# Lab-LVM/imagenet-models

Hardware: AMD Instinct MI355X
Metric: images/sec (whole node) GA-ConvNeXt-T 3x224x224 bf16 training step (higher is better)
Workload: dtype bf16; 1 GPU; ga_convnext_tiny_768 train step (fwd + GA loss lam=-0.8 + bwd + all-reduce + adamw lr=0), batch 256/GPU, drop_path 0.2, synthetic 3x224x224; global_batch=256, parallelism=dp1, dist_backend=none, grad_exchange=torch, allreduce_buckets=0

## Files before the change

imagenet-models_amd/_lib.py:

```python
import ctypes as C
import os

_HERE = os.path.dirname(os.path.abspath(__file__))
LIB_PATH = os.environ.get('GAEXT_LIB') or os.path.join(_HERE, 'csrc', 'libgaext.so')

GA_F32, GA_BF16 = 0, 1
ACT_NONE, ACT_GELU, ACT_RELU = 0, 1, 2
A_PLAIN, A_PATCH2, A_STEM4_NCHW, A_CONV3, A_CONV3S2, A_NEIGH2 = 0, 1, 2, 3, 4, 5
C_PLAIN, C_UNPATCH2 = 0, 1

vp, i32, i64, f32 = C.c_void_p, C.c_int, C.c_int64, C.c_float


class GemmDesc(C.Structure):
    _fields_ = [
        ('M', i32), ('N', i32), ('K', i32), ('batch', i32), ('dtype', i32),
        ('A', vp), ('lda', i64), ('strideA', i64), ('a_batch_mod', i32), ('a_kind', i32),
        ('a_H', i32), ('a_W', i32), ('a_C', i32), ('a_act', i32),
        ('B', vp), ('ldb', i64), ('strideB', i64),
        ('C', vp), ('ldc', i64), ('strideC', i64), ('c_kind', i32),
        ('c_H', i32), ('c_W', i32), ('c_C', i32), ('c_f32', i32), ('C2', vp), ('c2_mode', i32),
        ('alpha', f32), ('bias', vp), ('strideBias', i64), ('act', i32),
        ('H', vp), ('ldh', i64), ('strideH', i64), ('h_is_deriv', i32),
        ('rowscale', vp), ('rows_per_scale', i32),
# ... 173 lines not shown
    'ga_loss_dense_fwd_bwd': ([vp, vp, vp, vp, vp, vp, vp, i32, i32, i32, f32, i32, f32, f32, f32, i32, vp], i32),
    'ga_u8_normalize': ([vp, vp, i32, i32, i32, i32, C.POINTER(f32), C.POINTER(f32), vp], i32),
    'ga_input_erase': ([vp, i32, vp, i32, i32, i32, i32, C.POINTER(f32), C.POINTER(f32), vp, i32, i32, C.c_uint64, C.c_uint64, vp], i32),
    'ga_input_collate': ([vp, i32, vp, i32, i32, i32, i32, C.POINTER(f32), C.POINTER(f32), vp, vp, i32, i32, C.c_uint64, C.c_uint64, vp],
                         i32),
    'ga_mixup_target_elem': ([vp, vp, i32, i32, vp, C.c_double, vp], i32),
    'ga_mixup_batch': ([vp, vp, i32, i32, i32, i32, C.c_double, i32, i32, i32, i32, i32, vp], i32),
    'ga_mixup_target': ([vp, vp, i32, i32, C.c_double, C.c_double, vp], i32),
    'ga_agc_clip': ([vp, vp, vp, i32, f32, f32, vp], i32),
    'ga_small_linear_fwd': ([C.POINTER(SmallLinearDesc), vp], i32),
    'ga_small_linear_bwd': ([C.POINTER(SmallLinearDesc), vp, vp, i32, vp, vp, vp, vp], i32),
    'ga_colstats': ([vp, i64, i32, i32, vp, vp, i32, vp], i32),
    'ga_pad_copy_f32': ([vp, vp, i64, i64, i64, i64, i32, vp], i32),
    'ga_pad_copy': ([vp, vp, i64, i64, i64, i64, i32, i32, vp], i32),
    'ga_stem4_ln_fwd': ([vp, vp, i64, vp, vp, vp, vp, vp, vp, vp, i32, i32, i32, i32, f32, vp], i32),
    'ga_blockdiag_f32': ([vp, vp, i64, i32, i32, i32, i64, i32, i32, vp], i32),
    'ga_pad_groups_f32': ([vp, vp, i64, i64, i32, i32, i32, i32, i32, i32, vp], i32),
    'ga_attn_fwd': ([C.POINTER(AttnDesc), vp], i32),
    'ga_attn_bwd_workspace': ([C.POINTER(AttnDesc)], C.c_size_t),
    'ga_attn_bwd': ([C.POINTER(AttnDesc), vp, vp, vp, C.c_size_t, vp], i32),
    'ga_patchify': ([vp, vp, i32, i32, i32, i32, i32, i32, vp], i32),
    'ga_vit_embed_fwd': ([vp, vp, vp, vp, i32, i32, i32, i32, vp], i32),
    'ga_vit_embed_bwd': ([vp, vp, vp, vp, i32, i32, i32, i32, vp], i32),
    'ga_patchify_strided': ([vp, vp, i32, i32, i32, i32, i32, i32, i32, vp], i32),
    'ga_pos_add_fwd': ([vp, vp, vp, i32, i32, i32, i32, vp], i32),
    'ga_pos_add_bwd': ([vp, vp, i32, i32, i32, i32, vp], i32),
    'ga_dwpool_fwd': ([vp, vp, vp, vp, i32, i32, i32, i32, i32, i32, vp], i32),
    'ga_dwpool_bwd_data': ([vp, vp, vp, i32, i32, i32, i32, i32, i32, vp], i32),
    'ga_dwpool_bwd_weight': ([vp, vp, vp, vp, i32, i32, i32, i32, i32, i32, vp], i32),
    'ga_resize_concat_fwd': ([vp, vp, i32, i32, i32, i32, i32, i32, i64, i32, i32, vp], i32),
    'ga_resize_concat_bwd': ([vp, vp, i32, i32, i32, i32, i32, i32, i64, i32, i32, vp], i32),
    'ga_rows_bcast': ([vp, vp, i32, i32, i32, f32, i32, vp], i32),
    'ga_token_gap_fwd': ([vp, vp, i32, i32, i32, i32, vp], i32),
    'ga_token_gap_bwd': ([vp, vp, i32, i32, i32, i32, vp], i32),
    'ga_mlp_supported': ([i32, i32, i32], i32),
    'ga_mlp_fwd': ([C.POINTER(MlpDesc), vp], i32),
    'ga_mlp_bwd': ([C.POINTER(MlpBwdDesc), vp], i32),
    'ga_mlp_bwd_wgrad_supported': ([i32, i32, i32], i32),
    'ga_mlp_bwd_partials': ([C.POINTER(MlpBwdDesc)], C.c_size_t),
    'ga_memset': ([vp, i32, C.c_size_t, vp], i32),
    'ga_transpose_f32': ([vp, vp, i32, i32, i32, vp], i32),
    'ga_axpy_f32': ([vp, vp, f32, i64, vp], i32),
    'ga_lerp_f32': ([vp, vp, f32, i64, vp], i32),
    'ga_sumsq_f32': ([vp, i64, vp, vp], i32),
    'ga_lamb_stage1': ([vp, vp, vp, vp, vp, vp, vp, vp, i32, vp, vp], i32),
    'ga_lamb_stage2': ([vp, vp, vp, vp, i32, vp, vp], i32),
    'ga_clip_grad_f32': ([vp, i64, vp, f32, i32, vp], i32),
    'ga_rowscale': ([vp, vp, vp, i64, i64, i32, vp], i32),
    'ga_cast_from_f32': ([vp, vp, i64, i32, vp], i32),
    'ga_cast_to_f32': ([vp, vp, i64, i32, vp], i32),
}

_lib = None


def load():
    global _lib
    if _lib is not None:
        return _lib
    if not os.path.exists(LIB_PATH):
        raise RuntimeError(f'libgaext.so not found at {LIB_PATH}: build it with `make -C {os.path.dirname(LIB_PATH)}` '
                           f'(there is no CPU fallback for the product path)')
    lib = C.CDLL(LIB_PATH)
    for name, (argtypes, restype) in _SIGS.items():
        fn = getattr(lib, name)
        fn.argtypes = argtypes
        fn.restype = restype
    _lib = lib
    return lib


def last_error():
    buf = C.create_string_buffer(512)
    load().ga_last_error(buf, 512)
    return buf.value.decode(errors='replace')


def config_string():
    buf = C.create_string_buffer(1024)
    load().ga_config_string(buf, 1024)
    s = buf.value.decode(errors='replace')
    host = sorted(k for k in os.environ if k.startswith(('GAEXT_', 'GA_FUSED_MLP')) and k != 'GAEXT_LIB')
    known = {'GAEXT_ASYNC_WGRAD', 'GAEXT_FWD_SPLIT', 'GAEXT_PAR_BRANCH', 'GAEXT_FWD_SKEW', 'GAEXT_FUSE_DP', 'GAEXT_HEAD_STREAMS',
             'GA_FUSED_MLP', 'GAEXT_SMALL_SINGLE', 'GAEXT_SYNC_DEBUG', 'GAEXT_MLP_WG1'}
    for k in host:
        if k in known:
            s += f' host:{k}={os.environ[k]}'
    if os.environ.get('GAEXT_LIB'):
        s += f' lib={os.environ["GAEXT_LIB"]}'
    return s


class knobs:

    def __init__(self, **kv):
        self.kv = kv

    def __enter__(self):
        lib = load()
        for k, v in self.kv.items():
            check(lib.ga_set_knob(k.encode(), int(v)), f'ga_set_knob({k})')
        return self

    def __exit__(self, *exc):
        lib = load()
        for k in self.kv:
            lib.ga_unset_knob(k.encode())
        return False


def check(rc, what):
    if rc != 0:
        raise RuntimeError(f'libgaext {what} failed (code {rc}): {last_error()}')


def exported_symbols():
    return sorted(_SIGS)
```

imagenet-models_amd/csrc/gemm.hip:

```cpp
#include <stdlib.h>
#include <algorithm>
#include <type_traits>
#include "common.h"

namespace {

int num_cus() {
    static int n = [] {
        int c = 256;
        ga_device_info(&c, nullptr, nullptr);
        return c;
    }();
    return n;
}

constexpr int kThreads = 256;
constexpr int kRowBytes = 128;

__device__ __forceinline__ int xcd_remap(int bid, int nwg) {
    const int q = nwg >> 3, r = nwg & 7, xcd = bid & 7, idx = bid >> 3;
    return (xcd < r ? xcd * (q + 1) : r * (q + 1) + (xcd - r) * q) + idx;
}

struct RowCtx {
// ... 1471 lines not shown
        const int cur = (int)((s - s_begin) & 1);
        if (s + 1 < s_end) g_load(s + 1);
        const unsigned char* Ys = smem + cur * 32768;
        const unsigned char* Xs = Ys + 16384;
        if constexpr (sizeof(T) == 2) {
#pragma unroll
            for (int ks = 0; ks < 2; ++ks) {
                s16x4_t yf[4][2], xf[4][2];
#pragma unroll
                for (int hf = 0; hf < 2; ++hf) {
                    const int row = ks * 32 + 8 * (lane >> 4) + 4 * hf + ((lane & 15) >> 2);
                    const int sw = tn_swz(row);
#pragma unroll
                    for (int t = 0; t < 4; ++t) {
                        const int ch_y = ((wn * 64 + t * 16) >> 3) + ((lane & 3) >> 1);
                        const int ch_x = ((wk * 64 + t * 16) >> 3) + ((lane & 3) >> 1);
                        const unsigned ay = row * P::RB + ((ch_y ^ sw) << 4) + 8 * (lane & 1);
                        const unsigned ax = row * P::RB + ((ch_x ^ sw) << 4) + 8 * (lane & 1);
                        yf[t][hf] = __builtin_amdgcn_ds_read_tr16_b64_v4i16(
                            (__attribute__((address_space(3))) s16x4_t*)(Ys + ay));
                        xf[t][hf] = __builtin_amdgcn_ds_read_tr16_b64_v4i16(
                            (__attribute__((address_space(3))) s16x4_t*)(Xs + ax));
                    }
                }
#pragma unroll
                for (int tn = 0; tn < 4; ++tn)
#pragma unroll
                    for (int tk = 0; tk < 4; ++tk)
                        acc[tn][tk] = __builtin_amdgcn_mfma_f32_16x16x32_bf16(
                            *reinterpret_cast<const bf16x8_t*>(&yf[tn][0]), *reinterpret_cast<const bf16x8_t*>(&xf[tk][0]),
                            acc[tn][tk], 0, 0, 0);
            }
        } else {
#pragma unroll
            for (int ks = 0; ks < 8; ++ks) {
                const int row = ks * 4 + (lane >> 4);
                float yf[4], xf[4];
#pragma unroll
                for (int t = 0; t < 4; ++t) {
                    yf[t] = *reinterpret_cast<const float*>(Ys + row * P::RB + (wn * 64 + t * 16 + (lane & 15)) * 4);
                    xf[t] = *reinterpret_cast<const float*>(Xs + row * P::RB + (wk * 64 + t * 16 + (lane & 15)) * 4);
                }
#pragma unroll
                for (int tn = 0; tn < 4; ++tn)
#pragma unroll
                    for (int tk = 0; tk < 4; ++tk)
                        acc[tn][tk] = __builtin_amdgcn_mfma_f32_16x16x4f32(yf[tn], xf[tk], acc[tn][tk], 0, 0, 0);
            }
        }
        if (s + 1 < s_end) s_store(cur ^ 1);
        __syncthreads();
    }

    float* W = d.dW + z * d.strideW;
    const bool atomic = d.accumulate || d.split_m > 1;
#pragma unroll
    for (int tn = 0; tn < 4; ++tn)
#pragma unroll
        for (int tk = 0; tk < 4; ++tk)
#pragma unroll
            for (int r = 0; r < 4; ++r) {
                const int n = n0 + wn * 64 + tn * 16 + (lane >> 4) * 4 + r;
                const int k = k0 + wk * 64 + tk * 16 + (lane & 15);
                if (n < d.N && k < d.K) {
                    const float v = acc[tn][tk][r] * d.alpha;
                    if (atomic) atomicAdd(W + (long)n * d.ldw + k, v);
                    else W[(long)n * d.ldw + k] = v;
                }
            }
    if (do_bias) {
        float* red = reinterpret_cast<float*>(smem);
#pragma unroll
        for (int j = 0; j < EPC; ++j) red[rr * 128 + cc * EPC + j] = bsum[j];
        __syncthreads();
        if (tid < 128 && n0 + tid < d.N) {
            float s = 0.f;
            for (int r = 0; r < P::RSTEP; ++r) s += red[r * 128 + tid];
            atomicAdd(d.dbias + z * d.strideDbias + n0 + tid, s * d.alpha);
        }
    }
}

constexpr int kTn2Threads = 512, kTn2Stage = 32768, kTn2Smem = 4 * kTn2Stage;

template <bool P2>
__global__ __launch_bounds__(kTn2Threads) void gemm_tn2_kernel(const ga_wgrad_desc d, const int split_m,
                                                               float* __restrict__ part) {
    extern __shared__ __attribute__((aligned(16))) unsigned char smem[];
    const int tid = threadIdx.x, lane = tid & 63;
    const int wave = __builtin_amdgcn_readfirstlane(tid >> 6);
    const int wn = wave >> 2, wk = wave & 3;
    const int tiles_k = (d.K + 255) / 256, tiles_n = (d.N + 255) / 256;
    const int ntiles = tiles_k * tiles_n;
    const int bid = xcd_remap(blockIdx.x, ntiles * split_m);
    const int split = bid / ntiles, tile = bid - split * ntiles;
    const int tile_n = tile / tiles_k, tile_k = tile - tile_n * tiles_k;
    const int n0 = tile_n * 256, k0 = tile_k * 256;
    const int z = blockIdx.z;
    const int stages = d.M / 32;
    const int per = (stages + split_m - 1) / split_m;
    const int s_begin = split * per;
    const int s_end = s_begin + per < stages ? s_begin + per : stages;
    if (s_begin >= s_end) return;

    const int sub = wave >> 1;
    const bool is_y = sub < 2;
    const int ncols = is_y ? d.N : d.K;
    const int col0 = (is_y ? n0 : k0) + (sub & 1) * 128;
    const bool sub_live = col0 < ncols;
    const long ld = is_y ? d.ldy : d.ldx;
    const int zx = d.x_batch_mod > 0 ? z % d.x_batch_mod : z;
    const bf16_t* gsrc = is_y ? reinterpret_cast<const bf16_t*>(d.Y) + z * d.strideY
                              : reinterpret_cast<const bf16_t*>(d.X) + zx * d.strideX;
    const int lrow = 16 * (wave & 1) + (lane >> 4);
    const int pc = lane & 15;
    const bool xp2 = P2 && !is_y;
    const int sw_lo = ((lane >> 4) & 3) << 1;
    long goff[2];
#pragma unroll
    for (int b = 0; b < 2; ++b) {
        int c = col0 + ((pc ^ (sw_lo | (b << 3))) << 3);
        if (c >= ncols) c = 0;
        if (xp2) goff[b] = c + (c >= 2 * d.x_C ? (long)(d.x_W - 2) * d.x_C : 0);
        else goff[b] = (long)lrow * ld + c;
    }
    const unsigned lds0 = (unsigned)(size_t)(__attribute__((address_space(3))) unsigned char*)smem;
    const u32x4_s rs = make_rsrc(gsrc, xp2 ? (unsigned)(8L * d.M * d.x_C) : 0xffffffffu);
    unsigned voff[4];
    [[maybe_unused]] unsigned p2_ox[4];
    [[maybe_unused]] unsigned p2_ow = 1, p2_r = 0, p2_step = 0, p2_carry = 0;
    if (xp2) {
        p2_ow = (unsigned)d.x_W >> 1;
        const unsigned q = 32u / p2_ow, rowb = (unsigned)(d.x_W * d.x_C) * 2u;
        p2_r = 32u - q * p2_ow;
        p2_step = 128u * (unsigned)d.x_C + q * rowb;
        p2_carry = rowb;
#pragma unroll
        for (int i = 0; i < 4; ++i) {
            const unsigned m = (unsigned)s_begin * 32u + (unsigned)(lrow + 4 * i), t = m / p2_ow;
            p2_ox[i] = m - t * p2_ow;
            voff[i] = (unsigned)(((long)(2u * m + (unsigned)d.x_W * t)) * d.x_C + goff[(i >> 1) & 1]) * 2u;
        }
    } else {
#pragma unroll
        for (int i = 0; i < 4; ++i) voff[i] = (unsigned)(goff[(i >> 1) & 1] + (long)(4 * i) * ld) * 2u;
    }
    auto stage_load = [&](int s, int buf) __attribute__((always_inline)) {
        if (!sub_live) return;
        const unsigned soff = xp2 ? 0u : (unsigned)s * 64u * (unsigned)ld;
        const unsigned dst = lds0 + buf * kTn2Stage + sub * 8192 + (wave & 1) * 4096;
#pragma unroll
        for (int i = 0; i < 4; ++i) blds16(rs, voff[i], soff, dst + i * 1024);
        if constexpr (P2) {
            if (xp2) {
#pragma unroll
                for (int i = 0; i < 4; ++i) {
                    p2_ox[i] += p2_r;
                    const bool carry = p2_ox[i] >= p2_ow;
                    p2_ox[i] -= carry ? p2_ow : 0u;
                    voff[i] += p2_step + (carry ? p2_carry : 0u);
                }
            }
        }
    };

    int nv = (d.N - n0 - wn * 128 + 15) / 16; nv = nv < 0 ? 0 : (nv > 8 ? 8 : nv);
    int kv = (d.K - k0 - wk * 64 + 15) / 16;  kv = kv < 0 ? 0 : (kv > 4 ? 4 : kv);
    const bool do_bias = d.dbias != nullptr && tile_k == 0 && wk == 0;
    f32x4_t acc[8][4];
    float bsum[8];
#pragma unroll
    for (int i = 0; i < 8; ++i) {
        bsum[i] = 0.f;
#pragma unroll
        for (int j = 0; j < 4; ++j) acc[i][j] = f32x4_t{0.f, 0.f, 0.f, 0.f};
    }
    typedef __attribute__((ext_vector_type(2))) __bf16 bf16x2_t;
    const bf16x2_t ones2 = {(__bf16)1.0f, (__bf16)1.0f};

    const unsigned y_img = wn * 8192, x_img = 16384 + (wk >> 1) * 8192;
    const int xc0 = (wk & 1) * 8;
    unsigned yaddr[8], xaddr[4];
    {
        const int row = 8 * (lane >> 4) + ((lane & 15) >> 2);
        const int sw = tn_swz(row);
        const unsigned rb = row * 256 + 8 * (lane & 1);
#pragma unroll
        for (int t = 0; t < 8; ++t) yaddr[t] = y_img + rb + (((2 * t + ((lane & 3) >> 1)) ^ sw) << 4);
#pragma unroll
        for (int t = 0; t < 4; ++t) xaddr[t] = x_img + rb + (((xc0 + 2 * t + ((lane & 3) >> 1)) ^ sw) << 4);
    }
    auto compute = [&](int cur) {
        const unsigned char* st = smem + cur * kTn2Stage;
        s16x4_t yf[8][2], xf[4][2];
#pragma unroll
        for (int hf = 0; hf < 2; ++hf) {
#pragma unroll
            for (int t = 0; t < 4; ++t)
                xf[t][hf] = __builtin_amdgcn_ds_read_tr16_b64_v4i16(
                    (__attribute__((address_space(3))) s16x4_t*)(st + xaddr[t] + hf * 1024));
#pragma unroll
            for (int t = 0; t < 8; ++t)
                yf[t][hf] = __builtin_amdgcn_ds_read_tr16_b64_v4i16(
                    (__attribute__((address_space(3))) s16x4_t*)(st + yaddr[t] + hf * 1024));
        }
#pragma unroll
        for (int tn = 0; tn < 8; ++tn) {
            const bf16x8_t a = *reinterpret_cast<const bf16x8_t*>(&yf[tn][0]);
#pragma unroll
            for (int tk = 0; tk < 4; ++tk)
                acc[tn][tk] = __builtin_amdgcn_mfma_f32_16x16x32_bf16(
                    a, *reinterpret_cast<const bf16x8_t*>(&xf[tk][0]), acc[tn][tk], 0, 0, 0);
        }
        if (do_bias) {
#pragma unroll
            for (int tn = 0; tn < 8; ++tn) {
                const bf16x8_t a = *reinterpret_cast<const bf16x8_t*>(&yf[tn][0]);
#pragma unroll
                for (int j = 0; j < 4; ++j)
                    bsum[tn] = __builtin_amdgcn_fdot2_f32_bf16(bf16x2_t{a[2 * j], a[2 * j + 1]}, ones2, bsum[tn], false);
            }
        }
    };

    const int nst = s_end - s_begin;
#pragma unroll
    for (int j = 0; j < 3; ++j)
        if (j < nst) stage_load(s_begin + j, j);
    for (int it = 0; it < nst; ++it) {
        const int ahead = nst - 1 - it;
        if (ahead >= 2) asm volatile("s_waitcnt vmcnt(8)" ::: "memory");
        else if (ahead == 1) asm volatile("s_waitcnt vmcnt(4)" ::: "memory");
        else asm volatile("s_waitcnt vmcnt(0)" ::: "memory");
        __builtin_amdgcn_s_barrier();
        if (it + 3 < nst) stage_load(s_begin + it + 3, (it + 3) & 3);
        if (nv > 0 && kv > 0) compute(it & 3);
    }

    float* W = part ? part + ((long)z * split_m + split) * d.N * d.K : d.dW + z * d.strideW;
    const long ldw = part ? d.K : d.ldw;
    const float alpha = part ? 1.f : d.alpha;
    const bool atomic = !part && (d.accumulate || split_m > 1);
#pragma unroll
    for (int tn = 0; tn < 8; ++tn)
#pragma unroll
        for (int tk = 0; tk < 4; ++tk)
#pragma unroll
            for (int r = 0; r < 4; ++r) {
                const int n = n0 + wn * 128 + tn * 16 + (lane >> 4) * 4 + r;
                const int k = k0 + wk * 64 + tk * 16 + (lane & 15);
                if (n < d.N && k < d.K) {
                    const float v = acc[tn][tk][r] * alpha;
                    if (atomic) atomicAdd(W + (long)n * ldw + k, v);
                    else W[(long)n * ldw + k] = v;
                }
            }
    if (do_bias) {
#pragma unroll
        for (int tn = 0; tn < 8; ++tn) {
            float v = bsum[tn];
            v += __shfl_xor(v, 16, 64);
            v += __shfl_xor(v, 32, 64);
            const int n = n0 + wn * 128 + tn * 16 + lane;
            if (lane < 16 && n < d.N) atomicAdd(d.dbias + z * d.strideDbias + n, v * d.alpha);
        }
    }
}

__global__ __launch_bounds__(256) void tn2_reduce_kernel(const float* __restrict__ part, int nsplit, long nk, int K,
                                                         float alpha, float* __restrict__ dW, long ldw, long strideW) {
    const long z = blockIdx.y;
    const float* p = part + z * nsplit * nk;
    for (long i = ((long)blockIdx.x * 256 + threadIdx.x) * 4; i < nk; i += (long)gridDim.x * 1024) {
        float4 a = *reinterpret_cast<const float4*>(p + i);
#pragma unroll 4
        for (int s = 1; s < nsplit; ++s) {
            const float4 b = *reinterpret_cast<const float4*>(p + (long)s * nk + i);
            a.x += b.x; a.y += b.y; a.z += b.z; a.w += b.w;
        }
        const long n = i / K, k = i - n * K;
        float* dst = dW + z * strideW + n * ldw + k;
        dst[0] += alpha * a.x; dst[1] += alpha * a.y; dst[2] += alpha * a.z; dst[3] += alpha * a.w;
    }
}

bool tn2_eligible(const ga_wgrad_desc* d) {
    if (!(GA_KNOB("TN2", 1) && d->dtype == GA_BF16 && d->x_act == GA_ACT_NONE && d->M % 32 == 0 && d->M >= 8192 &&
          (d->accumulate || d->split_m > 1) && (long)d->M * d->ldy < (1L << 31)))
        return false;
    if (d->x_kind == GA_A_PLAIN) return (long)d->M * d->ldx < (1L << 31);
    if (d->x_kind == GA_A_PATCH2)
        return GA_KNOB("TN2_PATCH2", 1) && d->x_C > 0 && d->x_C % 8 == 0 && d->K == 4 * d->x_C && d->x_H > 0 && d->x_W > 0 &&
               d->x_H % 2 == 0 && d->x_W % 2 == 0 && d->M % ((long)(d->x_H / 2) * (d->x_W / 2)) == 0 &&
               8L * d->M * d->x_C < (1L << 31);
    return false;
}

size_t tn2_plan(const ga_wgrad_desc* d, int* split_out) {
    const int tiles = cdiv(d->N, 256) * cdiv(d->K, 256) * d->batch;
    const int stages = d->M / 32;
    const int wg_budget = GA_KNOB("TN2_WGS", 0);
    const int cus = wg_budget > 0 ? wg_budget : num_cus() * 3 / 4;
    int split = std::max(1, std::min(stages / 8, cus / tiles));
    split = cdiv(stages, cdiv(stages, split));
    *split_out = split;
    const long nk = (long)d->N * d->K;
    const long nk_min = GA_KNOB("TN2_PART_MIN", 65536);
    return (split > 1 && nk >= nk_min) ? (size_t)d->batch * split * nk * sizeof(float) : 0;
}

bool aligned16(const void* p) { return (reinterpret_cast<uintptr_t>(p) & 15) == 0; }

template <typename T, int TNW, int NWM, bool PLAIN, bool PRE, int EPI, bool DMA = false>
void launch_nt_(const ga_gemm_desc* d, hipStream_t s) {
    using CF = NTCfg<TNW, NWM>;
    constexpr int smem = DMA ? CF::SMEM_DMA : CF::SMEM;
    auto kern = gemm_nt_kernel<T, TNW, NWM, PLAIN, PRE, EPI, DMA>;
    static const int per_cu = [&] {
        int n = 0;
        if (smem > 65536 && hipFuncSetAttribute(reinterpret_cast<const void*>(kern),
                                                hipFuncAttributeMaxDynamicSharedMemorySize, smem) != hipSuccess)
            return 0;
        if (hipOccupancyMaxActiveBlocksPerMultiprocessor(&n, kern, CF::NTHR, smem) != hipSuccess || n < 1) n = 1;
        return n;
    }();
    if (per_cu == 0) {
        ga_set_error("ga_gemm: cannot reserve %d bytes of LDS", smem);
        return;
    }
    const int tiles = cdiv(d->M, CF::BM) * cdiv(d->N, CF::BN);
    const int cap = std::max(8, (per_cu * num_cus() / d->batch) / 8 * 8);
    dim3 grid(std::min(tiles, cap), 1, d->batch), block(CF::NTHR);
    hipLaunchKernelGGL(kern, grid, block, smem, s, *d);
}

template <int EPI>
void launch_nt_pp(const ga_gemm_desc* d, hipStream_t s) {
    auto kern = gemm_nt_pp_kernel<EPI>;
    static const bool ok = hipFuncSetAttribute(reinterpret_cast<const void*>(kern), hipFuncAttributeMaxDynamicSharedMemorySize, kPPSmem) == hipSuccess;
    if (!ok) {
        ga_set_error("ga_gemm: cannot reserve %d bytes of LDS", kPPSmem);
        return;
    }
    const int tiles = cdiv(d->M, 256) * cdiv(d->N, 256);
    const int cap = std::max(8, (num_cus() / d->batch) / 8 * 8);
    dim3 grid(std::min(tiles, cap), 1, d->batch), block(kPPThreads);
#ifdef GAEXT_DEBUG
    const int dbg = GA_KNOB("PP_DBG", 0);
#else
    const int dbg = 0;
#endif
    hipLaunchKernelGGL(kern, grid, block, kPPSmem, s, *d, dbg);
}

template <int EPI, int DBG = 0, int AK = 0>
void launch_nt_r3_(const ga_gemm_desc* d, hipStream_t s) {
    auto kern = gemm_nt_r3_kernel<EPI, DBG, AK>;
    static const bool ok = hipFuncSetAttribute(reinterpret_cast<const void*>(kern), hipFuncAttributeMaxDynamicSharedMemorySize, kR3Smem) == hipSuccess;
    if (!ok) {
        ga_set_error("ga_gemm: cannot reserve %d bytes of LDS", kR3Smem);
        return;
    }
    const int tiles = cdiv(d->M, 256) * cdiv(d->N, 128);
    const int cap = std::max(8, (2 * num_cus() / d->batch) / 8 * 8);
    dim3 grid(std::min(tiles, cap), 1, d->batch), block(kR3Threads);
    const int stagger = std::max(0, GA_KNOB("R3_STAGGER", 0));
    hipLaunchKernelGGL(kern, grid, block, kR3Smem, s, *d, stagger);
}
template <int EPI>
void launch_nt_r3(const ga_gemm_desc* d, hipStream_t s) {
#ifdef GAEXT_DEBUG
    switch (GA_KNOB("R3_DBG", 0)) {
        case 1: return launch_nt_r3_<EPI, 1>(d, s);
        case 2: return launch_nt_r3_<EPI, 2>(d, s);
        case 4: return launch_nt_r3_<EPI, 4>(d, s);
        case 6: return launch_nt_r3_<EPI, 6>(d, s);
        case 8: return launch_nt_r3_<EPI, 8>(d, s);
        case 10: return launch_nt_r3_<EPI, 10>(d, s);
        case 17: return launch_nt_r3_<EPI, 17>(d, s);
        case 33: return launch_nt_r3_<EPI, 33>(d, s);
        default: break;
    }
#endif
    launch_nt_r3_<EPI, 0>(d, s);
}

bool want_pp(const ga_gemm_desc* d, int epi);
bool want_r3(const ga_gemm_desc* d, int epi) {
    const int r3 = GA_KNOB("NT_R3", -1);
    const bool forced = r3 >= 0;
    const int mask = forced ? r3 : 15;
// ... 195 lines not shown
                default: launch_nt_<bf16_t, 4, 4, true, true, EPI_DG2, true>(d, s); break;
            }
        } else {
            switch (epi) {
                case EPI_PLAIN: launch_nt_<bf16_t, 3, 4, true, false, EPI_PLAIN, true>(d, s); break;
                case EPI_FC1: launch_nt_<bf16_t, 3, 4, true, false, EPI_FC1, true>(d, s); break;
                case EPI_FC2: launch_nt_<bf16_t, 3, 4, true, true, EPI_FC2, true>(d, s); break;
                default: launch_nt_<bf16_t, 3, 4, true, true, EPI_DG2, true>(d, s); break;
            }
        }
    } else if (want_pp(d, epi)) {
        switch (epi) {
            case EPI_PLAIN: launch_nt_pp<EPI_PLAIN>(d, s); break;
            case EPI_FC1: launch_nt_pp<EPI_FC1>(d, s); break;
            case EPI_FC2: launch_nt_pp<EPI_FC2>(d, s); break;
            default: launch_nt_pp<EPI_DG2>(d, s); break;
        }
    } else if (want_t256(d, epi)) {
        switch (epi) {
            case EPI_PLAIN: launch_nt_<bf16_t, 8, 4, true, false, EPI_PLAIN, true>(d, s); break;
            case EPI_FC1: launch_nt_<bf16_t, 8, 4, true, false, EPI_FC1, true>(d, s); break;
            case EPI_FC2: launch_nt_<bf16_t, 8, 4, true, false, EPI_FC2, true>(d, s); break;
            default: launch_nt_<bf16_t, 8, 4, true, false, EPI_DG2, true>(d, s); break;
        }
    } else if (tnw == 4 && want_dma2(d, epi)) {
        switch (epi) {
            case EPI_PLAIN: launch_nt_<bf16_t, 4, 2, true, false, EPI_PLAIN, true>(d, s); break;
            case EPI_FC1: launch_nt_<bf16_t, 4, 2, true, false, EPI_FC1, true>(d, s); break;
            case EPI_FC2: launch_nt_<bf16_t, 4, 2, true, true, EPI_FC2, true>(d, s); break;
            default: launch_nt_<bf16_t, 4, 2, true, true, EPI_DG2, true>(d, s); break;
        }
    } else if (tnw == 4) {
        if (want_big_tile(d, epi)) {
            if (epi == EPI_FC2) launch_nt_<bf16_t, 4, 4, true, true, EPI_FC2>(d, s);
            else launch_nt_<bf16_t, 4, 4, true, true, EPI_DG2>(d, s);
        } else {
            GA_LAUNCH_NT(4, 2);
        }
    } else if (tnw == 3) {
        GA_LAUNCH_NT(3, 2);
    } else {
        GA_LAUNCH_NT(2, 2);
    }
#undef GA_LAUNCH_NT
    return ga_check_launch("ga_gemm");
}

extern "C" int ga_wgrad(const ga_wgrad_desc* d, ga_stream_t stream) {
    GA_REQUIRE(d && d->Y && d->X && d->dW, "ga_wgrad: null operand");
    GA_REQUIRE(d->M > 0 && d->N > 0 && d->K > 0 && d->batch >= 1 && d->split_m >= 1, "ga_wgrad: bad shape");
    GA_REQUIRE(d->dtype == GA_F32 || d->dtype == GA_BF16, "ga_wgrad: bad dtype %d", d->dtype);
    const int epc = d->dtype == GA_BF16 ? 8 : 4;
    GA_REQUIRE(aligned16(d->Y) && aligned16(d->X), "ga_wgrad: operands must be 16-byte aligned");
    GA_REQUIRE(d->N % epc == 0 && d->ldy % epc == 0 && d->strideY % epc == 0, "ga_wgrad: N/ldy must be multiples of %d",
               epc);
    if (d->x_kind == GA_A_PLAIN) {
        GA_REQUIRE(d->ldx % epc == 0 && d->strideX % epc == 0 && d->ldx >= (d->K + epc - 1) / epc * epc,
                   "ga_wgrad: ldx must be a multiple of %d and cover K rounded up", epc);
    } else if (d->x_kind == GA_A_PATCH2) {
        GA_REQUIRE(d->x_C % epc == 0 && d->K == 4 * d->x_C, "ga_wgrad: PATCH2 needs K==4C");
    } else if (d->x_kind == GA_A_CONV3) {
        GA_REQUIRE(d->x_C % epc == 0 && d->K == 9 * d->x_C, "ga_wgrad: CONV3 needs K==9C");
    } else if (d->x_kind == GA_A_CONV3S2) {
        GA_REQUIRE(d->x_C % epc == 0 && d->K == 9 * d->x_C, "ga_wgrad: CONV3S2 needs K==9C");
    } else if (d->x_kind == GA_A_NEIGH2) {
        GA_REQUIRE(d->x_C % epc == 0 && d->K == 4 * d->x_C, "ga_wgrad: NEIGH2 needs K==4C");
    } else if (d->x_kind == GA_A_STEM4_NCHW) {
        GA_REQUIRE(d->x_C == 3 && d->K == 48, "ga_wgrad: STEM4 needs C=3,K=48");
    } else {
        GA_REQUIRE(false, "ga_wgrad: bad x_kind %d", d->x_kind);
    }
    hipStream_t s = reinterpret_cast<hipStream_t>(stream);
    if (d->x_kind == GA_A_CONV3 && ga_conv3_c64_wgrad_try(d, s)) return ga_check_launch("ga_wgrad");
    if (d->x_kind == GA_A_CONV3S2 && d->x_C == 64 && ga_conv3s2_c64_wgrad_try(d, s)) return ga_check_launch("ga_wgrad");
    if (d->x_kind == GA_A_CONV3S2 && d->x_C == 8 && ga_conv0_c8_wgrad_try(d, s)) return ga_check_launch("ga_wgrad");
    if (d->x_kind == GA_A_STEM4_NCHW && ga_stem4_wgrad_try(d, s)) return ga_check_launch("ga_wgrad");
    if (tn2_eligible(d)) {
        const bool p2 = d->x_kind == GA_A_PATCH2;
        static const bool attr_ok = hipFuncSetAttribute(reinterpret_cast<const void*>(gemm_tn2_kernel<false>),
                                                        hipFuncAttributeMaxDynamicSharedMemorySize, kTn2Smem) == hipSuccess &&
                                    hipFuncSetAttribute(reinterpret_cast<const void*>(gemm_tn2_kernel<true>),
                                                        hipFuncAttributeMaxDynamicSharedMemorySize, kTn2Smem) == hipSuccess;
        GA_REQUIRE(attr_ok, "ga_wgrad: cannot reserve %d bytes of LDS", kTn2Smem);
        int split;
        const size_t need = tn2_plan(d, &split);
        dim3 grid2(cdiv(d->N, 256) * cdiv(d->K, 256) * split, 1, d->batch), block2(kTn2Threads);
        float* part = (need && d->workspace && (size_t)d->ws_bytes >= need) ? reinterpret_cast<float*>(d->workspace) : nullptr;
        GA_REQUIRE(!part || aligned16(part), "ga_wgrad: workspace must be 16-byte aligned");
        const long nk = (long)d->N * d->K;
        if (p2) hipLaunchKernelGGL(gemm_tn2_kernel<true>, grid2, block2, kTn2Smem, s, *d, split, part);
        else hipLaunchKernelGGL(gemm_tn2_kernel<false>, grid2, block2, kTn2Smem, s, *d, split, part);
        if (part)
            hipLaunchKernelGGL(tn2_reduce_kernel, dim3((unsigned)std::min<long>(2048, cdiv(nk, 1024)), d->batch), dim3(256),
                               0, s, part, split, nk, d->K, d->alpha, d->dW, d->ldw, d->strideW);
        return ga_check_launch("ga_wgrad");
    }
    dim3 grid(cdiv(d->N, 128) * cdiv(d->K, 128) * d->split_m, 1, d->batch), block(kThreads);
    if (d->dtype == GA_BF16)
        hipLaunchKernelGGL(gemm_tn_kernel<bf16_t>, grid, block, 65536, s, *d);
    else
        hipLaunchKernelGGL(gemm_tn_kernel<float>, grid, block, 65536, s, *d);
    return ga_check_launch("ga_wgrad");
}

extern "C" size_t ga_wgrad_workspace(const ga_wgrad_desc* d) {
    if (!d || d->M <= 0 || d->N <= 0 || d->K <= 0 || d->batch < 1) return 0;
    if (d->x_kind == GA_A_CONV3 || (d->x_kind == GA_A_CONV3S2 && (d->x_C == 64 || d->x_C == 8))) return ga_conv3_c64_wgrad_workspace(d);
    if (d->x_kind == GA_A_STEM4_NCHW) return ga_stem4_wgrad_workspace(d);
    if (!tn2_eligible(d)) return 0;
    int split;
    return tn2_plan(d, &split);
}
```

Measured before the change: 10880 images/sec.

## Plan ragged wgrad tiles with per-class split-M and tile-local partial buffers

Reworks the tn2 weight-gradient GEMM planner so that ragged edge tiles (half-empty in K or N) form separate classes with their own cost-weighted split-M factor. A binary search balances workgroups against the CU budget. Partials are now stored per workgroup in 256x256 slots, optionally in raw accumulator fragment order to skip scattered stores. The reduce kernel is rewritten to map slots back to dW. Wave roles can be permuted on ragged tiles to balance work. This adds planner complexity and a larger workspace (full slots per workgroup).

```diff
diff --git a/imagenet-models_amd/_lib.py b/imagenet-models_amd/_lib.py
--- a/imagenet-models_amd/_lib.py
+++ b/imagenet-models_amd/_lib.py
@@ -279,7 +279,7 @@
     s = buf.value.decode(errors='replace')
     host = sorted(k for k in os.environ if k.startswith(('GAEXT_', 'GA_FUSED_MLP')) and k != 'GAEXT_LIB')
     known = {'GAEXT_ASYNC_WGRAD', 'GAEXT_FWD_SPLIT', 'GAEXT_PAR_BRANCH', 'GAEXT_FWD_SKEW', 'GAEXT_FUSE_DP', 'GAEXT_HEAD_STREAMS',
-             'GA_FUSED_MLP', 'GAEXT_SMALL_SINGLE', 'GAEXT_SYNC_DEBUG', 'GAEXT_MLP_WG1'}
+             'GA_FUSED_MLP', 'GAEXT_SMALL_SINGLE', 'GAEXT_SYNC_DEBUG', 'GAEXT_MLP_WG1', 'GAEXT_TN2_RAGGED', 'GAEXT_TN2_PART_ACC'}
     for k in host:
         if k in known:
             s += f' host:{k}={os.environ[k]}'
diff --git a/imagenet-models_amd/csrc/gemm.hip b/imagenet-models_amd/csrc/gemm.hip
--- a/imagenet-models_amd/csrc/gemm.hip
+++ b/imagenet-models_amd/csrc/gemm.hip
@@ -1577,26 +1577,50 @@
 }
 
 constexpr int kTn2Threads = 512, kTn2Stage = 32768, kTn2Smem = 4 * kTn2Stage;
+constexpr int kTn2Slot = 256 * 256;
+
+struct Tn2Cls { int wg0, tiles, split, per; };
+struct Tn2Plan {
+    Tn2Cls c[4];
+    int nwg;
+    int rk, rn;
+    int roles;
+    int part_acc;
+};
 
 template <bool P2>
-__global__ __launch_bounds__(kTn2Threads) void gemm_tn2_kernel(const ga_wgrad_desc d, const int split_m,
+__global__ __launch_bounds__(kTn2Threads) void gemm_tn2_kernel(const ga_wgrad_desc d, const Tn2Plan p,
                                                                float* __restrict__ part) {
     extern __shared__ __attribute__((aligned(16))) unsigned char smem[];
     const int tid = threadIdx.x, lane = tid & 63;
     const int wave = __builtin_amdgcn_readfirstlane(tid >> 6);
-    const int wn = wave >> 2, wk = wave & 3;
     const int tiles_k = (d.K + 255) / 256, tiles_n = (d.N + 255) / 256;
-    const int ntiles = tiles_k * tiles_n;
-    const int bid = xcd_remap(blockIdx.x, ntiles * split_m);
-    const int split = bid / ntiles, tile = bid - split * ntiles;
-    const int tile_n = tile / tiles_k, tile_k = tile - tile_n * tiles_k;
+    const int bid = xcd_remap(blockIdx.x, p.nwg);
+    int ci = 0, wg0 = p.c[0].wg0, ctiles = p.c[0].tiles, csplit = p.c[0].split, per = p.c[0].per;
+#pragma unroll
+    for (int c = 1; c < 4; ++c)
+        if (p.c[c].tiles > 0 && bid >= p.c[c].wg0) {
+            ci = c; wg0 = p.c[c].wg0; ctiles = p.c[c].tiles; csplit = p.c[c].split; per = p.c[c].per;
+        }
+    const int split = (bid - wg0) / ctiles, ct = bid - wg0 - split * ctiles;
+    const int tkf = tiles_k - p.rk, tnf = tiles_n - p.rn;
+    const int cw = (ci & 1) ? 1 : tkf;
+    const int tile_n = ct / cw + ((ci & 2) ? tnf : 0), tile_k = ct % cw + ((ci & 1) ? tkf : 0);
     const int n0 = tile_n * 256, k0 = tile_k * 256;
     const int z = blockIdx.z;
     const int stages = d.M / 32;
-    const int per = (stages + split_m - 1) / split_m;
     const int s_begin = split * per;
     const int s_end = s_begin + per < stages ? s_begin + per : stages;
     if (s_begin >= s_end) return;
+    int role = wave;
+    {
+        const bool kr = d.K - k0 <= 128, nr = d.N - n0 <= 128;
+        const int perm = kr ? (p.roles & 3) : nr ? ((p.roles >> 2) & 3) : 0;
+        if (perm == 1) role = (wave & 1) | ((wave & 2) << 1) | ((wave & 4) >> 1);
+        else if (perm == 2) role = (wave & 4) | ((wave & 1) << 1) | ((wave >> 1) & 1);
+        else if (perm == 3) role = (wave >> 1) | ((wave & 1) << 2);
+    }
+    const int wn = role >> 2, wk = role & 3;
 
     const int sub = wave >> 1;
     const bool is_y = sub < 2;
@@ -1732,24 +1756,34 @@
         if (nv > 0 && kv > 0) compute(it & 3);
     }
 
-    float* W = part ? part + ((long)z * split_m + split) * d.N * d.K : d.dW + z * d.strideW;
-    const long ldw = part ? d.K : d.ldw;
-    const float alpha = part ? 1.f : d.alpha;
-    const bool atomic = !part && (d.accumulate || split_m > 1);
-#pragma unroll
-    for (int tn = 0; tn < 8; ++tn)
-#pragma unroll
-        for (int tk = 0; tk < 4; ++tk)
-#pragma unroll
-            for (int r = 0; r < 4; ++r) {
-                const int n = n0 + wn * 128 + tn * 16 + (lane >> 4) * 4 + r;
-                const int k = k0 + wk * 64 + tk * 16 + (lane & 15);
-                if (n < d.N && k < d.K) {
-                    const float v = acc[tn][tk][r] * alpha;
-                    if (atomic) atomicAdd(W + (long)n * ldw + k, v);
-                    else W[(long)n * ldw + k] = v;
-                }
-            }
+    if (part && p.part_acc) {
+        f32x4_t* dst = reinterpret_cast<f32x4_t*>(part + ((long)z * p.nwg + bid) * kTn2Slot + role * 8192) + lane;
+#pragma unroll
+        for (int tn = 0; tn < 8; ++tn)
+#pragma unroll
+            for (int tk = 0; tk < 4; ++tk)
+                if (tn < nv && tk < kv) dst[(tn * 4 + tk) * 64] = acc[tn][tk];
+    } else {
+        float* W = part ? part + ((long)z * p.nwg + bid) * kTn2Slot : d.dW + z * d.strideW;
+        const long ldw = part ? 256 : d.ldw;
+        const int nb = part ? n0 : 0, kb = part ? k0 : 0;
+        const float alpha = part ? 1.f : d.alpha;
+        const bool atomic = !part && (d.accumulate || csplit > 1);
+#pragma unroll
+        for (int tn = 0; tn < 8; ++tn)
+#pragma unroll
+            for (int tk = 0; tk < 4; ++tk)
+#pragma unroll
+                for (int r = 0; r < 4; ++r) {
+                    const int n = n0 + wn * 128 + tn * 16 + (lane >> 4) * 4 + r;
+                    const int k = k0 + wk * 64 + tk * 16 + (lane & 15);
+                    if (n < d.N && k < d.K) {
+                        const float v = acc[tn][tk][r] * alpha;
+                        if (atomic) atomicAdd(W + (long)(n - nb) * ldw + (k - kb), v);
+                        else W[(long)(n - nb) * ldw + (k - kb)] = v;
+                    }
+                }
+    }
     if (do_bias) {
 #pragma unroll
         for (int tn = 0; tn < 8; ++tn) {
@@ -1762,20 +1796,47 @@
     }
 }
 
-__global__ __launch_bounds__(256) void tn2_reduce_kernel(const float* __restrict__ part, int nsplit, long nk, int K,
+__global__ __launch_bounds__(256) void tn2_reduce_kernel(const float* __restrict__ part, const Tn2Plan p, int N, int K,
                                                          float alpha, float* __restrict__ dW, long ldw, long strideW) {
     const long z = blockIdx.y;
-    const float* p = part + z * nsplit * nk;
-    for (long i = ((long)blockIdx.x * 256 + threadIdx.x) * 4; i < nk; i += (long)gridDim.x * 1024) {
-        float4 a = *reinterpret_cast<const float4*>(p + i);
+    const int tile = blockIdx.x >> 6, q = (blockIdx.x & 63) * 256 + threadIdx.x;
+    const int tiles_k = (K + 255) / 256, tiles_n = (N + 255) / 256;
+    const int tile_n = tile / tiles_k, tile_k = tile - tile_n * tiles_k;
+    int row, col;
+    if (p.part_acc) {
+        const int lane = q & 63, tk = (q >> 6) & 3, tn = (q >> 8) & 7, wk = (q >> 11) & 3, wn = q >> 13;
+        row = wn * 128 + tn * 16 + (lane >> 4) * 4; col = wk * 64 + tk * 16 + (lane & 15);
+    } else {
+        row = q >> 6; col = (q & 63) * 4;
+    }
+    const int n = tile_n * 256 + row, k = tile_k * 256 + col;
+    if (n >= N || k >= K) return;
+    const int tkf = tiles_k - p.rk, tnf = tiles_n - p.rn;
+    const int ci = (tile_k >= tkf ? 1 : 0) | (tile_n >= tnf ? 2 : 0);
+    int wg0 = p.c[0].wg0, ctiles = p.c[0].tiles, csplit = p.c[0].split;
+#pragma unroll
+    for (int c = 1; c < 4; ++c)
+        if (ci == c) { wg0 = p.c[c].wg0; ctiles = p.c[c].tiles; csplit = p.c[c].split; }
+    const int ct = (tile_n - ((ci & 2) ? tnf : 0)) * ((ci & 1) ? 1 : tkf) + (tile_k - ((ci & 1) ? tkf : 0));
+    const float* src = part + (z * p.nwg + wg0 + ct) * kTn2Slot + q * 4;
+    float4 a = *reinterpret_cast<const float4*>(src);
 #pragma unroll 4
-        for (int s = 1; s < nsplit; ++s) {
-            const float4 b = *reinterpret_cast<const float4*>(p + (long)s * nk + i);
-            a.x += b.x; a.y += b.y; a.z += b.z; a.w += b.w;
-        }
-        const long n = i / K, k = i - n * K;
-        float* dst = dW + z * strideW + n * ldw + k;
+    for (int s = 1; s < csplit; ++s) {
+        const float4 b = *reinterpret_cast<const float4*>(src + (long)s * ctiles * kTn2Slot);
+        a.x += b.x; a.y += b.y; a.z += b.z; a.w += b.w;
+    }
+    float* dst = dW + z * strideW + n * ldw + k;
+    const float v[4] = {a.x, a.y, a.z, a.w};
+    if (p.part_acc) {
+#pragma unroll
+        for (int j = 0; j < 4; ++j)
+            if (n + j < N) dst[j * ldw] += alpha * v[j];
+    } else if (k + 3 < K) {
         dst[0] += alpha * a.x; dst[1] += alpha * a.y; dst[2] += alpha * a.z; dst[3] += alpha * a.w;
+    } else {
+#pragma unroll
+        for (int j = 0; j < 3; ++j)
+            if (k + j < K) dst[j] += alpha * v[j];
     }
 }
 
@@ -1791,17 +1852,61 @@
     return false;
 }
 
-size_t tn2_plan(const ga_wgrad_desc* d, int* split_out) {
-    const int tiles = cdiv(d->N, 256) * cdiv(d->K, 256) * d->batch;
+size_t tn2_plan(const ga_wgrad_desc* d, Tn2Plan* p) {
+    const int tiles_n = cdiv(d->N, 256), tiles_k = cdiv(d->K, 256);
     const int stages = d->M / 32;
     const int wg_budget = GA_KNOB("TN2_WGS", 0);
-    const int cus = wg_budget > 0 ? wg_budget : num_cus() * 3 / 4;
-    int split = std::max(1, std::min(stages / 8, cus / tiles));
-    split = cdiv(stages, cdiv(stages, split));
-    *split_out = split;
+    const int cus = (wg_budget > 0 ? wg_budget : num_cus() * 3 / 4) / d->batch;
+    const bool ragged = GA_KNOB("TN2_RAGGED", 1) != 0;
+    p->rk = ragged && d->K - (tiles_k - 1) * 256 <= 128;
+    p->rn = ragged && d->N - (tiles_n - 1) * 256 <= 128;
+    p->roles = ragged ? (GA_KNOB("TN2_ROLE_K", 1) & 3) | (GA_KNOB("TN2_ROLE_N", 0) & 3) << 2 : 0;
+    const int tkf = tiles_k - p->rk, tnf = tiles_n - p->rn;
+    int ntile[4] = {tnf * tkf, tnf * p->rk, p->rn * tkf, p->rn * p->rk};
+    const int cost[4] = {8, GA_KNOB("TN2_COST_K", 6), GA_KNOB("TN2_COST_N", 6), GA_KNOB("TN2_COST_NK", 6)};
+    const int max_split = std::max(1, stages / 8);
+    const int min_per = cdiv(stages, max_split);
+    int per[4] = {0, 0, 0, 0};
+    auto wgs_at = [&](long t) {
+        long n = 0;
+        for (int c = 0; c < 4; ++c) {
+            if (!ntile[c]) continue;
+            per[c] = (int)std::min<long>(stages, std::max<long>(min_per, t / std::max(1, cost[c])));
+            n += (long)ntile[c] * cdiv(stages, per[c]);
+        }
+        return n;
+    };
+    const int per_u = cdiv(stages, std::max(1, std::min(max_split, cus / (tiles_n * tiles_k))));
+    long t_u = 0, t_w = 0;
+    for (int c = 0; c < 4; ++c)
+        if (ntile[c]) t_u = std::max(t_u, (long)per_u * cost[c]);
+    if (ntile[0] != tiles_n * tiles_k) {
+        long lo = 1, hi = 8L * stages;
+        while (lo < hi) {
+            const long mid = (lo + hi) / 2;
+            if (wgs_at(mid) <= cus) hi = mid; else lo = mid + 1;
+        }
+        wgs_at(lo);
+        for (int c = 0; c < 4; ++c)
+            if (ntile[c]) t_w = std::max(t_w, (long)per[c] * cost[c]);
+    }
+    if (t_w == 0 || t_w * 16 > t_u * 15) {
+        p->rk = p->rn = 0;
+        ntile[0] = tiles_n * tiles_k; ntile[1] = ntile[2] = ntile[3] = 0;
+        per[0] = per_u;
+    }
+    int nwg = 0, max_s = 1;
+    for (int c = 0; c < 4; ++c) {
+        const int split = ntile[c] ? cdiv(stages, per[c]) : 0;
+        p->c[c] = Tn2Cls{nwg, ntile[c], split, per[c]};
+        nwg += ntile[c] * split;
+        max_s = std::max(max_s, split);
+    }
+    p->nwg = nwg;
+    p->part_acc = GA_KNOB("TN2_PART_ACC", 1) != 0;
     const long nk = (long)d->N * d->K;
     const long nk_min = GA_KNOB("TN2_PART_MIN", 65536);
-    return (split > 1 && nk >= nk_min) ? (size_t)d->batch * split * nk * sizeof(float) : 0;
+    return (max_s > 1 && nk >= nk_min) ? (size_t)d->batch * nwg * kTn2Slot * sizeof(float) : 0;
 }
 
 bool aligned16(const void* p) { return (reinterpret_cast<uintptr_t>(p) & 15) == 0; }
@@ -2163,17 +2268,16 @@
                                     hipFuncSetAttribute(reinterpret_cast<const void*>(gemm_tn2_kernel<true>),
                                                         hipFuncAttributeMaxDynamicSharedMemorySize, kTn2Smem) == hipSuccess;
         GA_REQUIRE(attr_ok, "ga_wgrad: cannot reserve %d bytes of LDS", kTn2Smem);
-        int split;
-        const size_t need = tn2_plan(d, &split);
-        dim3 grid2(cdiv(d->N, 256) * cdiv(d->K, 256) * split, 1, d->batch), block2(kTn2Threads);
+        Tn2Plan tp;
+        const size_t need = tn2_plan(d, &tp);
+        dim3 grid2(tp.nwg, 1, d->batch), block2(kTn2Threads);
         float* part = (need && d->workspace && (size_t)d->ws_bytes >= need) ? reinterpret_cast<float*>(d->workspace) : nullptr;
         GA_REQUIRE(!part || aligned16(part), "ga_wgrad: workspace must be 16-byte aligned");
-        const long nk = (long)d->N * d->K;
-        if (p2) hipLaunchKernelGGL(gemm_tn2_kernel<true>, grid2, block2, kTn2Smem, s, *d, split, part);
-        else hipLaunchKernelGGL(gemm_tn2_kernel<false>, grid2, block2, kTn2Smem, s, *d, split, part);
+        if (p2) hipLaunchKernelGGL(gemm_tn2_kernel<true>, grid2, block2, kTn2Smem, s, *d, tp, part);
+        else hipLaunchKernelGGL(gemm_tn2_kernel<false>, grid2, block2, kTn2Smem, s, *d, tp, part);
         if (part)
-            hipLaunchKernelGGL(tn2_reduce_kernel, dim3((unsigned)std::min<long>(2048, cdiv(nk, 1024)), d->batch), dim3(256),
-                               0, s, part, split, nk, d->K, d->alpha, d->dW, d->ldw, d->strideW);
+            hipLaunchKernelGGL(tn2_reduce_kernel, dim3(cdiv(d->N, 256) * cdiv(d->K, 256) * 64, d->batch), dim3(256), 0, s, part,
+                               tp, d->N, d->K, d->alpha, d->dW, d->ldw, d->strideW);
         return ga_check_launch("ga_wgrad");
     }
     dim3 grid(cdiv(d->N, 128) * cdiv(d->K, 128) * d->split_m, 1, d->batch), block(kThreads);
@@ -2189,6 +2293,6 @@
     if (d->x_kind == GA_A_CONV3 || (d->x_kind == GA_A_CONV3S2 && (d->x_C == 64 || d->x_C == 8))) return ga_conv3_c64_wgrad_workspace(d);
     if (d->x_kind == GA_A_STEM4_NCHW) return ga_stem4_wgrad_workspace(d);
     if (!tn2_eligible(d)) return 0;
-    int split;
-    return tn2_plan(d, &split);
-}
+    Tn2Plan tp;
+    return tn2_plan(d, &tp);
+}
```

Result: no change. 10840 images/sec (-0.3%).
